# limuhit/pseudocylindrical_convolution

Hardware: AMD Instinct MI355X
Metric: ERP MPix/s enc+dec, 4096x2048 model-idx 3 (higher is better)
Workload: dtype f32; 1 GPU; ERP 4096x2048 encode+decode, model-idx 3 --ssim (valid_dim 56), 8 frame(s)/GPU/step; frames_per_gpu=8, parallelism=frames sharded, no data-path collective, weights=seeded random (transforms seed 1234, entropy randn*0.05 seed 7), content=smooth, cores_per_rank=16

## Files before the change

pseudocylindrical_convolution_amd/csrc/wino42.hip:

```cpp
#include <atomic>
#include <stdlib.h>
#include <type_traits>
#include "conv_host.h"

namespace {

#ifdef PCONV_W42_STAMP
__device__ unsigned long long w42_stamps[8][6];
#define W42_STAMP(var) const unsigned long long var = __builtin_readcyclecounter()
#else
#define W42_STAMP(var)
#endif

typedef float f32x16 __attribute__((ext_vector_type(16)));
typedef float f32x2 __attribute__((ext_vector_type(2)));
typedef __attribute__((address_space(3))) void lds_ptr_t;
typedef const __attribute__((address_space(1))) void glb_ptr_t;
typedef const __attribute__((address_space(1))) char glb_bytes_t;

constexpr int kThreads = 512, kWaves = 8;
constexpr int XW = 3;
constexpr int NXI = kWaves * XW;
constexpr int TX = 32, TY = 2;
constexpr int OROWS = 4 * TY, OCOLS = 2 * TX;
constexpr int CO = 64;
constexpr int KC = 4;
constexpr int PR = OROWS + 2, PC = OCOLS + 2;
constexpr int PSZ = KC * PR * PC;
constexpr int PLD = (PSZ + kThreads - 1) / kThreads;
constexpr int PBUF = PLD * kThreads;
constexpr int PRING = 2;
constexpr int NT = TX * TY;
constexpr int VSZ = NXI * KC * NT;
constexpr int USZ = KC * XW * CO;
constexpr int URING = 3;
constexpr int ULD = USZ / 4 / 64;
constexpr int UNROLL = 6;
constexpr int kStageFloats = PRING * PBUF + 2 * VSZ + kWaves * URING * USZ;
constexpr int kLdsFloats = kStageFloats + 256;
constexpr int ESZ = NXI * 16 * 32;
static_assert(2 * ESZ <= kStageFloats, "the two exchange buffers fit the stage memory");
static_assert(kLdsFloats * 4 <= 160 * 1024, "LDS of a CU");
static_assert(PSZ <= PBUF && USZ % 256 == 0, "stage sizes");
static_assert(PLD + 2 * ULD < 64, "vmcnt counts to 63");
static_assert(KC == 4 && NXI == 24, "transform: waves 0-3 take one channel of the stage each; three GEMMs per wave");

__global__ void wino42_pack_kernel(const float *__restrict__ w, float *__restrict__ upk, int cout, int cin, int cin_pad,
                                   int cblocks) {
  const long long total = (long long)cblocks * cin_pad * CO;
  const long long i = (long long)blockIdx.x * blockDim.x + threadIdx.x;
  if (i >= total) return;
  const int j = (int)(i % CO);
  const int ci = (int)((i / CO) % cin_pad);
  const int cb = (int)(i / ((long long)CO * cin_pad));
  const int co = cb * CO + j;
  float g[3][3];
#pragma unroll
  for (int a = 0; a < 3; a++)
#pragma unroll
    for (int b = 0; b < 3; b++) g[a][b] = (co < cout && ci < cin) ? w[(((size_t)co * cin + ci) * 3 + a) * 3 + b] : 0.f;
  float r[6][3];
#pragma unroll
  for (int b = 0; b < 3; b++) {
    const float g0 = g[0][b], g1 = g[1][b], g2 = g[2][b];
    r[0][b] = g0 * 0.25f;
    r[1][b] = (g0 + g1 + g2) * (-1.f / 6.f);
    r[2][b] = (g0 - g1 + g2) * (-1.f / 6.f);
    r[3][b] = g0 * (1.f / 24.f) + g1 * (1.f / 12.f) + g2 * (1.f / 6.f);
    r[4][b] = g0 * (1.f / 24.f) - g1 * (1.f / 12.f) + g2 * (1.f / 6.f);
    r[5][b] = g2;
  }
#pragma unroll
  for (int a = 0; a < 6; a++) {
    const float u[4] = {r[a][0], (r[a][0] + r[a][1] + r[a][2]) * 0.5f, (r[a][0] - r[a][1] + r[a][2]) * 0.5f, r[a][2]};
#pragma unroll
    for (int b = 0; b < 4; b++) {
      const int xi = a * 4 + b;
      upk[((((size_t)cb * kWaves + xi / XW) * cin_pad + ci) * XW + (xi % XW)) * CO + j] = u[b];
    }
  }
}

template <int OFF>
__device__ __forceinline__ float w42_lds_read(unsigned addr) {
  static_assert(OFF >= 0 && OFF < 65536, "ds_read offset field is 16 bits");
  float v;
  asm volatile("ds_read_b32 %0, %1 offset:%2" : "=v"(v) : "v"(addr), "n"(OFF));
  return v;
}

template <int PENDING>
__device__ __forceinline__ void w42_wait(float (&a)[2], float (&b)[2]) {
  asm volatile("s_waitcnt lgkmcnt(%4)" : "+v"(a[0]), "+v"(a[1]), "+v"(b[0]), "+v"(b[1]) : "n"(PENDING));
}

template <int U, int VB, int ST>
__device__ __forceinline__ void w42_read_step(float (&a)[2], float (&b)[2], unsigned abase, unsigned bbase) {
  constexpr int x = ST >> 1, kp = ST & 1;
  constexpr int aoff = (U * USZ + (kp * 2 * XW + x) * CO) * 4;
  constexpr int boff = (VB * VSZ + (x * KC + kp * 2) * NT) * 4;
  a[0] = w42_lds_read<aoff>(abase);
  a[1] = w42_lds_read<aoff + 128>(abase);
  b[0] = w42_lds_read<boff>(bbase);
  b[1] = w42_lds_read<boff + 128>(bbase);
}

struct W42Half {
  const float *tp;
  float *tv;
  float cf[3][5];
};
struct W42Rows {
  float t[5][4];
};
template <int PB>
__device__ __forceinline__ void w42_half_load(const W42Half &h, W42Rows &w) {
  const float *p = h.tp + PB * PBUF;
#pragma unroll
  for (int a = 0; a < 5; a++) {
    const f32x2 lo = *reinterpret_cast<const f32x2 *>(p + a * PC), hi = *reinterpret_cast<const f32x2 *>(p + a * PC + 2);
    w.t[a][0] = lo.x, w.t[a][1] = lo.y, w.t[a][2] = hi.x, w.t[a][3] = hi.y;
  }
}
__device__ __forceinline__ void w42_half_horizontal(W42Rows &w) {
#pragma unroll
  for (int a = 0; a < 5; a++) {
    const float d0 = w.t[a][0], d1 = w.t[a][1], d2 = w.t[a][2], d3 = w.t[a][3];
    w.t[a][0] = d0 - d2, w.t[a][1] = d1 + d2, w.t[a][2] = d2 - d1, w.t[a][3] = d1 - d3;
  }
}
template <int VBUF, int R>
__device__ __forceinline__ void w42_half_row(const W42Half &h, const W42Rows &w) {
  constexpr int XS = KC * NT;
  float *v = h.tv + VBUF * VSZ + R * 4 * XS;
#pragma unroll
  for (int j = 0; j < 4; j++) {
    float s = h.cf[R][4] * w.t[4][j];
    s = __builtin_fmaf(h.cf[R][3], w.t[3][j], s);
    s = __builtin_fmaf(h.cf[R][2], w.t[2][j], s);
    s = __builtin_fmaf(h.cf[R][1], w.t[1][j], s);
    s = __builtin_fmaf(h.cf[R][0], w.t[0][j], s);
    v[j * XS] = s;
  }
}

template <int U, int VB, int ST, bool IL, class PD, class WD>
__device__ __forceinline__ void w42_mma_steps(f32x16 (&acc)[XW][2][2], float (&a)[2][2], float (&b)[2][2], unsigned abase,
                                              unsigned bbase, const W42Half &h, W42Rows &rows, PD &pd, WD &wd) {
  constexpr int NST = 2 * XW;
  constexpr int X = ST >> 1, S = ST & 1;
  static_assert(NST == 6, "the transform pieces are placed by hand in six steps");
  if constexpr (ST + 1 < NST) w42_read_step<U, VB, ST + 1>(a[(ST + 1) & 1], b[(ST + 1) & 1], abase, bbase);
  w42_wait<(ST + 1 < NST) ? 4 : 0>(a[S], b[S]);
  __builtin_amdgcn_sched_barrier(0);
  using std::integral_constant;
  auto dma = [&](auto g_c) {
    constexpr int G = decltype(g_c)::value;
    if constexpr (IL && ST <= 1 && ST * 3 + G < PLD && G < 3) {
      __builtin_amdgcn_sched_barrier(0);
      pd(integral_constant<int, ST * 3 + G>{});
      __builtin_amdgcn_sched_barrier(0);
    }
    if constexpr (IL && ST == NST - 1 && G < ULD) {
      __builtin_amdgcn_sched_barrier(0);
      wd(integral_constant<int, G>{});
      __builtin_amdgcn_sched_barrier(0);
    }
  };
  acc[X][0][0] = __builtin_amdgcn_mfma_f32_32x32x2f32(a[S][0], b[S][0], acc[X][0][0], 0, 0, 0);
  if constexpr (ST == 0) {
    __builtin_amdgcn_sched_barrier(0);
    w42_half_load<VB ^ 1>(h, rows);
    __builtin_amdgcn_sched_barrier(0);
  }
  if constexpr (ST == 1) {
    __builtin_amdgcn_sched_barrier(0);
    w42_half_horizontal(rows);
    __builtin_amdgcn_sched_barrier(0);
  }
  dma(integral_constant<int, 0>{});
  acc[X][0][1] = __builtin_amdgcn_mfma_f32_32x32x2f32(a[S][0], b[S][1], acc[X][0][1], 0, 0, 0);
  dma(integral_constant<int, 1>{});
  acc[X][1][0] = __builtin_amdgcn_mfma_f32_32x32x2f32(a[S][1], b[S][0], acc[X][1][0], 0, 0, 0);
  if constexpr (ST >= 2 && ST <= 4) {
    __builtin_amdgcn_sched_barrier(0);
    w42_half_row<VB ^ 1, ST - 2>(h, rows);
    __builtin_amdgcn_sched_barrier(0);
  }
  dma(integral_constant<int, 2>{});
  acc[X][1][1] = __builtin_amdgcn_mfma_f32_32x32x2f32(a[S][1], b[S][1], acc[X][1][1], 0, 0, 0);
  __builtin_amdgcn_sched_barrier(0);
  if constexpr (ST + 1 < NST) w42_mma_steps<U, VB, ST + 1, IL>(acc, a, b, abase, bbase, h, rows, pd, wd);
}

template <bool RES, bool D2W>
__global__ __launch_bounds__(kThreads) void wino42_conv3x3_kernel(
    const float *__restrict__ in, const float *__restrict__ upk, float *out, int cin, int cin_pad, int h,
    int w, int cout, int ho, int wo, int tiles_r, int tiles_c, int cblocks, WView vin, WView vout, WEpilogue ep) {
  W42_STAMP(st_start);
  extern __shared__ float lds[];
  float *Ps = lds, *Vs = lds + PRING * PBUF, *Us = lds + PRING * PBUF + 2 * VSZ;

  int b = blockIdx.x;
  const int cb = b % cblocks;
  b /= cblocks;
  const int trx = b % tiles_r;
  b /= tiles_r;
  const int tcx = b % tiles_c;
  const int t = b / tiles_c;
  const int r0 = trx * OROWS, c0 = tcx * OCOLS, cout0 = cb * CO;

  const int tid = threadIdx.x;
  const int lane = tid & 63;
  const int wave = __builtin_amdgcn_readfirstlane(tid >> 6);
  const int l31 = lane & 31, half = lane >> 5;
  float *outp = out + (size_t)t * vout.ts;
  const int limit = ep.col_limit ? ep.col_limit[t % ep.npart] : wo;

  if (c0 >= limit) {
    for (int e = tid; e < CO * OROWS * OCOLS; e += kThreads) {
      const int col = e % OCOLS, row = (e / OCOLS) % OROWS, co = cout0 + e / (OCOLS * OROWS);
      if (co < cout && r0 + row < ho && c0 + col < wo) {
        if (D2W)
          outp[(size_t)(co >> 2) * vout.cs + (size_t)(2 * (r0 + row) + ((co >> 1) & 1)) * vout.rs + 2 * (c0 + col) + (co & 1)] = 0.f;
        else
          outp[(size_t)co * vout.cs + (size_t)(r0 + row) * vout.rs + c0 + col] = 0.f;
      }
    }
    return;
  }

  const float *inp = in + (size_t)t * vin.ts;
  const int nchunk = cin_pad / KC;

  unsigned xoffs[PLD];
#pragma unroll
  for (int j = 0; j < PLD; j++) {
    int e = tid + j * kThreads;
    e = e < PSZ ? e : 0;
    const int pc = e % PC, pr = (e / PC) % PR, ci = e / (PC * PR);
    int ir = r0 + pr, ic = c0 + pc;
    ir = ir < h ? ir : h - 1;
    ic = ic < w ? ic : w - 1;
    xoffs[j] = (unsigned)(((long long)ci * vin.cs + (long long)ir * vin.rs + ic) * 4);
  }
  const size_t xstep = (size_t)KC * vin.cs;
  auto patch_piece = [&](int chunk, int buf, int j) {
    unsigned xo = xoffs[j];
    asm volatile("" : "+v"(xo));
    glb_bytes_t *xb = (glb_bytes_t *)(inp + chunk * xstep);
    __builtin_amdgcn_global_load_lds((glb_ptr_t *)(xb + xo), (lds_ptr_t *)(Ps + buf * PBUF + j * kThreads + wave * 64), 4, 0,
                                     0);
  };
  auto issue_patch = [&](int chunk, int buf, bool guard) {
    if (guard && chunk >= nchunk) return;
#pragma unroll
    for (int j = 0; j < PLD; j++) patch_piece(chunk, buf, j);
  };
  const float *uw = upk + ((size_t)cb * kWaves + wave) * cin_pad * XW * CO;
  float *us_w = Us + wave * URING * USZ;
  auto weight_piece = [&](int chunk, auto j_c) {
    constexpr int j = decltype(j_c)::value;
    glb_bytes_t *src = (glb_bytes_t *)(uw + (size_t)chunk * USZ);
    float *dst = us_w + (chunk % URING) * USZ;
    unsigned lo = (unsigned)lane * 16u;
    asm volatile("" : "+v"(lo));
    __builtin_amdgcn_global_load_lds((glb_ptr_t *)(src + lo), (lds_ptr_t *)dst, 16, j * 1024, 0);
  };
  auto issue_weights = [&](int chunk, bool guard) {
    if (guard && chunk >= nchunk) return;
    static_assert(ULD == 3, "weight pieces are issued by name");
    weight_piece(chunk, std::integral_constant<int, 0>{});
    weight_piece(chunk, std::integral_constant<int, 1>{});
    weight_piece(chunk, std::integral_constant<int, 2>{});
  };

  const int wave4 = wave >> 2, tch = wave & 3;
  const int tty = lane >> 5, ttx = lane & 31;
  const float *tp0 = Ps + (tch * PR + 4 * tty + wave4) * PC + 2 * ttx;
  float *tv0 = Vs + (wave4 * 12 * KC + tch) * NT + lane;
  const W42Half half_t = {tp0, tv0,
                          {{wave4 ? -2.f : 4.f, wave4 ? -1.f : 0.f, wave4 ? 2.f : -5.f, wave4 ? 1.f : 0.f, wave4 ? 0.f : 1.f},
                           {wave4 ? 2.f : 0.f, wave4 ? -1.f : -4.f, wave4 ? -2.f : -4.f, 1.f, wave4 ? 0.f : 1.f},
                           {wave4 ? 4.f : 0.f, wave4 ? 0.f : 4.f, wave4 ? -5.f : -4.f, wave4 ? 0.f : -1.f, 1.f}}};
  auto transform_full = [&](int pbuf, int vbuf) {
    W42Rows rows;
    const float *p = tp0 + pbuf * PBUF;
#pragma unroll
    for (int a = 0; a < 5; a++) {
      const f32x2 lo = *reinterpret_cast<const f32x2 *>(p + a * PC), hi = *reinterpret_cast<const f32x2 *>(p + a * PC + 2);
      rows.t[a][0] = lo.x, rows.t[a][1] = lo.y, rows.t[a][2] = hi.x, rows.t[a][3] = hi.y;
    }
    w42_half_horizontal(rows);
    constexpr int XS = KC * NT;
    float *v = tv0 + vbuf * VSZ;
#pragma unroll
    for (int r = 0; r < 3; r++)
#pragma unroll
      for (int j = 0; j < 4; j++) {
        float s = half_t.cf[r][4] * rows.t[4][j];
        s = __builtin_fmaf(half_t.cf[r][3], rows.t[3][j], s);
        s = __builtin_fmaf(half_t.cf[r][2], rows.t[2][j], s);
        s = __builtin_fmaf(half_t.cf[r][1], rows.t[1][j], s);
        s = __builtin_fmaf(half_t.cf[r][0], rows.t[0][j], s);
        v[(r * 4 + j) * XS] = s;
      }
  };

  f32x16 acc[XW][2][2];
#pragma unroll
  for (int x = 0; x < XW; x++)
#pragma unroll
    for (int m = 0; m < 2; m++)
#pragma unroll
      for (int n = 0; n < 2; n++)
#pragma unroll
        for (int r = 0; r < 16; r++) acc[x][m][n][r] = 0.f;

  float *Bt = lds + kStageFloats;
  if (wave < 4) {
    const float *src = wave < 2 ? ep.bias : (ep.act == 1 ? ep.slope : nullptr);
    int co = cout0 + (wave & 1) * 64 + lane;
    co = co < cout ? co : cout - 1;
    if (src)
      __builtin_amdgcn_global_load_lds((glb_ptr_t *)(src + co), (lds_ptr_t *)(Bt + wave * 64), 4, 0, 0);
    else
      Bt[wave * 64 + lane] = 0.f;
  }
  issue_patch(0, 0, true);
#pragma unroll
  for (int k = 0; k < URING; k++) issue_weights(k, true);
  issue_patch(1, 1, true);
  __builtin_amdgcn_s_waitcnt(0);
  __syncthreads();
  transform_full(0, 0);

  const unsigned lds0 = (unsigned)reinterpret_cast<uintptr_t>(lds);
  const unsigned abase = lds0 + (unsigned)((us_w - lds) + half * XW * CO + l31) * 4u;
  const unsigned bbase = lds0 + (unsigned)((Vs - lds) + ((wave * XW) * KC + half) * NT + l31) * 4u;

#ifdef PCONV_W42_STAMP
  unsigned long long st_bar = 0, st_n = 0;
#endif
  W42_STAMP(st_prologue);
  auto body = [&](auto us_c, auto vb_c, auto steady_c, int chunk) {
    constexpr int US = decltype(us_c)::value;
    constexpr int vb = decltype(vb_c)::value;
    constexpr bool STEADY = decltype(steady_c)::value;
    W42_STAMP(tb0);
    if (STEADY)
      asm volatile("s_waitcnt vmcnt(%0) lgkmcnt(0)\n\ts_barrier" ::"n"(ULD) : "memory");
    else
      asm volatile("s_waitcnt vmcnt(0) lgkmcnt(0)\n\ts_barrier" ::: "memory");
#ifdef PCONV_W42_STAMP
    if (STEADY) st_bar += __builtin_readcyclecounter() - tb0, st_n += 1;
#endif
    if (!STEADY) issue_patch(chunk + 2, vb, true);
    float a[2][2], bv[2][2];
    W42Rows rows;
    w42_read_step<US, vb, 0>(a[0], bv[0], abase, bbase);
    auto pd = [&](auto j_c) {
      constexpr int J = decltype(j_c)::value;
      if (J * kThreads + wave * 64 >= PSZ) return;
      patch_piece(chunk + 2, vb, J);
    };
    auto wd = [&](auto j_c) { weight_piece(chunk + URING, j_c); };
    w42_mma_steps<US, vb, 0, STEADY>(acc, a, bv, abase, bbase, half_t, rows, pd, wd);
    asm volatile("s_waitcnt lgkmcnt(0)" ::: "memory");
    if (!STEADY) issue_weights(chunk + URING, true);
  };
  using std::integral_constant;
  auto group = [&](auto steady_c, int c6) {
    body(integral_constant<int, 0>{}, integral_constant<int, 0>{}, steady_c, c6);
    body(integral_constant<int, 1>{}, integral_constant<int, 1>{}, steady_c, c6 + 1);
    body(integral_constant<int, 2>{}, integral_constant<int, 0>{}, steady_c, c6 + 2);
    body(integral_constant<int, 0>{}, integral_constant<int, 1>{}, steady_c, c6 + 3);
    body(integral_constant<int, 1>{}, integral_constant<int, 0>{}, steady_c, c6 + 4);
    body(integral_constant<int, 2>{}, integral_constant<int, 1>{}, steady_c, c6 + 5);
  };
  int c6 = 0;
#pragma unroll 1
  for (; c6 + 2 * UNROLL <= nchunk; c6 += UNROLL) group(integral_constant<bool, true>{}, c6);
#pragma unroll 1
  for (; c6 < nchunk; c6 += UNROLL) group(integral_constant<bool, false>{}, c6);
  W42_STAMP(st_loop);
  __syncthreads();

  const int act = ep.act;
  const int trim_at = ep.trim ? limit : wo;
  const float *resp = RES ? ep.residual + (size_t)t * ep.vres.ts : nullptr;
  const int co16 = tid >> 5, etx = tid & 31;
  const int ocol = c0 + 2 * etx;
  struct ResBlock {
    f32x2 v[4];
  };
  auto load_res = [&](int k) {
    ResBlock rb = {{{0.f, 0.f}, {0.f, 0.f}, {0.f, 0.f}, {0.f, 0.f}}};
    if (RES && k < 8) {
      const int m = k >> 2, n = (k >> 1) & 1, hq = k & 1;
      const int oc = ocol < wo ? ocol : wo - 2;
      int co = cout0 + m * 32 + hq * 16 + co16;
      co = co < cout ? co : cout - 1;
#pragma unroll
      for (int a2 = 0; a2 < 4; a2++) {
        int rr = r0 + 4 * n + a2;
        rr = rr < ho ? rr : ho - 1;
        rb.v[a2] = *reinterpret_cast<const f32x2 *>(resp + (size_t)co * ep.vres.cs + (size_t)rr * ep.vres.rs + oc);
      }
    }
    return rb;
  };
  ResBlock rq[2] = {load_res(0), load_res(1)};
#pragma unroll
  for (int k = 0; k < 8; k++) {
    const int m = k >> 2, n = (k >> 1) & 1, hq = k & 1;
    float *Es = lds + (k & 1) * ESZ;
    const ResBlock rcur = rq[k & 1];
    rq[k & 1] = load_res(k + 2);
#pragma unroll
    for (int x = 0; x < XW; x++) {
      float *e = Es + ((wave * XW + x) * 16 + 4 * half) * 32 + l31;
#pragma unroll
      for (int rl = 0; rl < 8; rl++) e[((rl & 3) + 8 * (rl >> 2)) * 32] = acc[x][m][n][8 * hq + rl];
    }
    asm volatile("s_waitcnt lgkmcnt(0)\n\ts_barrier" ::: "memory");
    float mm[NXI];
#pragma unroll
    for (int xi = 0; xi < NXI; xi++) mm[xi] = Es[(xi * 16 + co16) * 32 + etx];
    const int row = m * 32 + hq * 16 + co16;
    const int co = cout0 + row;
    const int orow = r0 + 4 * n;
    if (co < cout && ocol < wo) {
      float s[6][2];
#pragma unroll
      for (int i = 0; i < 6; i++) {
        s[i][0] = mm[4 * i] + mm[4 * i + 1] + mm[4 * i + 2];
        s[i][1] = mm[4 * i + 1] - mm[4 * i + 2] - mm[4 * i + 3];
      }
      float y[4][2];
#pragma unroll
      for (int c = 0; c < 2; c++) {
        const float p12 = s[1][c] + s[2][c], m12 = s[1][c] - s[2][c];
        const float p34 = s[3][c] + s[4][c], m34 = s[3][c] - s[4][c];
        y[0][c] = s[0][c] + p12 + p34;
        y[1][c] = __builtin_fmaf(2.f, m34, m12);
        y[2][c] = __builtin_fmaf(4.f, p34, p12);
        y[3][c] = __builtin_fmaf(8.f, m34, m12) + s[5][c];
      }
      const float bco = Bt[row], sl = Bt[128 + row];
#pragma unroll
      for (int a2 = 0; a2 < 4; a2++) {
        if (orow + a2 >= ho) continue;
        float y0 = y[a2][0] + bco, y1 = y[a2][1] + bco;
        if (act == 1) {
          y0 = y0 < 0 ? y0 * sl : y0;
          y1 = y1 < 0 ? y1 * sl : y1;
        }
        if (RES) {
          y0 = rcur.v[a2].x + y0;
          y1 = rcur.v[a2].y + y1;
        }
        if (!D2W) {
          if (ocol >= trim_at) y0 = 0.f;
          if (ocol + 1 >= trim_at) y1 = 0.f;
          float *q = outp + (size_t)co * vout.cs + (size_t)(orow + a2) * vout.rs + ocol;
          f32x2 yv = {y0, y1};
          *reinterpret_cast<f32x2 *>(q) = yv;
        } else {
          float *q = outp + (size_t)(co >> 2) * vout.cs + (size_t)(2 * (orow + a2) + ((co >> 1) & 1)) * vout.rs + 2 * ocol +
                     (co & 1);
          q[0] = y0;
          q[2] = y1;
        }
      }
    }
  }
#ifdef PCONV_W42_STAMP
  if (blockIdx.x == gridDim.x / 2 + 1 && lane == 0) {
    unsigned long long *o = w42_stamps[wave];
    o[0] = st_start, o[1] = st_prologue, o[2] = st_loop, o[3] = __builtin_readcyclecounter(), o[4] = st_bar, o[5] = st_n;
  }
#endif
}

}

#ifdef PCONV_W42_STAMP
extern "C" int pconv_wino42_read_stamps(unsigned long long *out) {
  return hipMemcpyFromSymbol(out, HIP_SYMBOL(w42_stamps), sizeof(w42_stamps)) == hipSuccess ? 0 : 1;
}
#endif

extern "C" long long pconv_wino42_packed_size(int cout, int cin) {
  const int cblocks = (cout + CO - 1) / CO, cin_pad = (cin + KC - 1) / KC * KC;
  return (long long)cblocks * NXI * cin_pad * CO;
}

extern "C" int pconv_wino42_pack_weight(const float *w, float *packed, int cout, int cin, void *stream) {
  PCONV_REQUIRE(w && packed && cout > 0 && cin > 0, "wino42_pack: bad argument");
  const int cblocks = (cout + CO - 1) / CO, cin_pad = (cin + KC - 1) / KC * KC;
  const long long total = (long long)cblocks * cin_pad * CO;
  hipLaunchKernelGGL(wino42_pack_kernel, dim3((unsigned)((total + 255) / 256)), dim3(256), 0, as_stream(stream), w, packed,
                     cout, cin, cin_pad, cblocks);
  PCONV_LAUNCH_CHECK("wino42_pack_weight");
  return PCONV_OK;
}

extern "C" int pconv_wino42_supported(int cin, int h, int w, int cout, int d2w) {
  if (h < 6 || w < 4 || ((w - 2) & 1)) return 0;
  if (cin < 24 || cin % 24 || cout < 32) return 0;
  if (d2w && (cout & 3)) return 0;
  return 1;
}

extern "C" int pconv_conv3x3_wino42(const float *in, const float *packed_u, const float *bias, float *out, int tn, int cin,
                                    int h, int w, int cout, int act, const float *slope, const int32_t *col_limit,
                                    int npart, const float *residual, int trim, int d2w, const long long *views,
                                    void *stream) {
  WView vin, vout;
  WEpilogue ep;
  if (int rc = wino_check_args("conv3x3_wino42", pconv_wino42_supported, KC, true, in, packed_u, bias, out, cin, h, w, cout,
                               act, slope, col_limit, npart, residual, trim, d2w, views, &vin, &vout, &ep))
    return rc;
  const int ho = h - 2, wo = w - 2;
  const int tiles_r = (ho + OROWS - 1) / OROWS, tiles_c = (wo + OCOLS - 1) / OCOLS;
  const int cblocks = (cout + CO - 1) / CO, cin_pad = (cin + KC - 1) / KC * KC;
  const long long grid = (long long)tn * tiles_r * tiles_c * cblocks;
  PCONV_REQUIRE(grid > 0 && grid <= 0x7fffffffLL, "conv3x3_wino42: grid %lld out of range", grid);
  const size_t smem = (size_t)kLdsFloats * sizeof(float);
  using kernel_t = decltype(&wino42_conv3x3_kernel<false, false>);
  static const kernel_t kernels[3] = {wino42_conv3x3_kernel<false, false>, wino42_conv3x3_kernel<true, false>,
                                      wino42_conv3x3_kernel<false, true>};
  const int kind = d2w ? 2 : (residual ? 1 : 0);
  static std::atomic<unsigned long long> raised[3];
  if (int rc = pconv_raise_lds(kernels[kind], smem, raised[kind], "conv3x3_wino42")) return rc;
  hipLaunchKernelGGL(kernels[kind], dim3((unsigned)grid), dim3(kThreads), smem, as_stream(stream), in, packed_u, out, cin,
                     cin_pad, h, w, cout, ho, wo, tiles_r, tiles_c, cblocks, vin, vout, ep);
  PCONV_LAUNCH_CHECK("conv3x3_wino42");
  return PCONV_OK;
}
```

Measured before the change: 95.63 MPix/s.

## Add wide 128-output-channel Winograd F(4,3) tile variant for cout divisible by 128

Result: slower. 94.47 MPix/s (-1.2%).

```diff
diff --git a/pseudocylindrical_convolution_amd/csrc/wino42.hip b/pseudocylindrical_convolution_amd/csrc/wino42.hip
--- a/pseudocylindrical_convolution_amd/csrc/wino42.hip
+++ b/pseudocylindrical_convolution_amd/csrc/wino42.hip
@@ -6,7 +6,7 @@
 namespace {
 
 #ifdef PCONV_W42_STAMP
-__device__ unsigned long long w42_stamps[8][6];
+__device__ unsigned long long w42_stamps[2][8][6];
 #define W42_STAMP(var) const unsigned long long var = __builtin_readcyclecounter()
 #else
 #define W42_STAMP(var)
@@ -21,32 +21,55 @@
 constexpr int kThreads = 512, kWaves = 8;
 constexpr int XW = 3;
 constexpr int NXI = kWaves * XW;
-constexpr int TX = 32, TY = 2;
-constexpr int OROWS = 4 * TY, OCOLS = 2 * TX;
-constexpr int CO = 64;
+constexpr int TY = 2;
+constexpr int OROWS = 4 * TY;
+constexpr int BCOLS = 64;
 constexpr int KC = 4;
-constexpr int PR = OROWS + 2, PC = OCOLS + 2;
-constexpr int PSZ = KC * PR * PC;
-constexpr int PLD = (PSZ + kThreads - 1) / kThreads;
-constexpr int PBUF = PLD * kThreads;
+constexpr int PR = OROWS + 2;
 constexpr int PRING = 2;
-constexpr int NT = TX * TY;
-constexpr int VSZ = NXI * KC * NT;
-constexpr int USZ = KC * XW * CO;
-constexpr int URING = 3;
-constexpr int ULD = USZ / 4 / 64;
-constexpr int UNROLL = 6;
-constexpr int kStageFloats = PRING * PBUF + 2 * VSZ + kWaves * URING * USZ;
+constexpr int ESZ = NXI * 16 * 32;
+
+template <bool WIDE>
+struct W42Geom {
+  static constexpr int CO = WIDE ? 128 : 64;
+  static constexpr int TX = WIDE ? 16 : 32;
+  static constexpr int MT = CO / 32, NB = TX * TY / 32;
+  static constexpr int OCOLS = 2 * TX;
+  static constexpr int PC = OCOLS + 2;
+  static constexpr int PSZ = KC * PR * PC;
+  static constexpr int PLD = (PSZ + kThreads - 1) / kThreads;
+  static constexpr int PBUF = PLD * kThreads;
+  static constexpr int NT = TX * TY;
+  static constexpr int VSZ = NXI * KC * NT;
+  static constexpr int USZ = KC * XW * CO;
+  static constexpr int URING = WIDE ? 2 : 3;
+  static constexpr int ULD = USZ / 4 / 64;
+  static constexpr int UNROLL = WIDE ? 2 : 6;
+  static constexpr int kStageFloats = PRING * PBUF + 2 * VSZ + kWaves * URING * USZ;
+  static_assert(MT * NB == 4, "four MFMAs per step");
+  static_assert(2 * ESZ <= kStageFloats, "the two exchange buffers fit the stage memory");
+  static_assert(PSZ <= PBUF && USZ % 256 == 0 && ULD % 3 == 0, "stage sizes");
+  static_assert(PLD <= 6 && PLD + 2 * ULD < 64, "patch pieces fit two steps; vmcnt counts to 63");
+};
+constexpr int kStageFloats = W42Geom<false>::kStageFloats;
 constexpr int kLdsFloats = kStageFloats + 256;
-constexpr int ESZ = NXI * 16 * 32;
-static_assert(2 * ESZ <= kStageFloats, "the two exchange buffers fit the stage memory");
+static_assert(W42Geom<true>::kStageFloats <= kStageFloats, "one LDS size for both shapes");
 static_assert(kLdsFloats * 4 <= 160 * 1024, "LDS of a CU");
-static_assert(PSZ <= PBUF && USZ % 256 == 0, "stage sizes");
-static_assert(PLD + 2 * ULD < 64, "vmcnt counts to 63");
 static_assert(KC == 4 && NXI == 24, "transform: waves 0-3 take one channel of the stage each; three GEMMs per wave");
 
+__host__ __device__ inline int w42_wide_blocks(int cout) { return cout % 128 == 0 ? cout / 128 : 0; }
+struct W42Slice {
+  size_t off;
+  int pitch;
+};
+__host__ __device__ inline W42Slice w42_slice64(int cb, int nwide, int cin_pad) {
+  if (nwide) return {(size_t)(cb >> 1) * NXI * cin_pad * 128 + (size_t)(cb & 1) * 64, 128};
+  return {(size_t)cb * NXI * cin_pad * 64, 64};
+}
+
 __global__ void wino42_pack_kernel(const float *__restrict__ w, float *__restrict__ upk, int cout, int cin, int cin_pad,
-                                   int cblocks) {
+                                   int cblocks, int nwide) {
+  constexpr int CO = 64;
   const long long total = (long long)cblocks * cin_pad * CO;
   const long long i = (long long)blockIdx.x * blockDim.x + threadIdx.x;
   if (i >= total) return;
@@ -54,6 +77,7 @@
   const int ci = (int)((i / CO) % cin_pad);
   const int cb = (int)(i / ((long long)CO * cin_pad));
   const int co = cb * CO + j;
+  const W42Slice sl = w42_slice64(cb, nwide, cin_pad);
   float g[3][3];
 #pragma unroll
   for (int a = 0; a < 3; a++)
@@ -76,7 +100,7 @@
 #pragma unroll
     for (int b = 0; b < 4; b++) {
       const int xi = a * 4 + b;
-      upk[((((size_t)cb * kWaves + xi / XW) * cin_pad + ci) * XW + (xi % XW)) * CO + j] = u[b];
+      upk[sl.off + (((size_t)(xi / XW) * cin_pad + ci) * XW + (xi % XW)) * sl.pitch + j] = u[b];
     }
   }
 }
@@ -93,131 +117,186 @@
 __device__ __forceinline__ void w42_wait(float (&a)[2], float (&b)[2]) {
   asm volatile("s_waitcnt lgkmcnt(%4)" : "+v"(a[0]), "+v"(a[1]), "+v"(b[0]), "+v"(b[1]) : "n"(PENDING));
 }
-
-template <int U, int VB, int ST>
-__device__ __forceinline__ void w42_read_step(float (&a)[2], float (&b)[2], unsigned abase, unsigned bbase) {
+template <int PENDING>
+__device__ __forceinline__ void w42_wait(float (&a)[4], float (&b)[1]) {
+  asm volatile("s_waitcnt lgkmcnt(%5)" : "+v"(a[0]), "+v"(a[1]), "+v"(a[2]), "+v"(a[3]), "+v"(b[0]) : "n"(PENDING));
+}
+
+template <bool WIDE, int U, int VB, int ST>
+__device__ __forceinline__ void w42_read_step(float (&a)[W42Geom<WIDE>::MT], float (&b)[W42Geom<WIDE>::NB], unsigned abase,
+                                              unsigned bbase) {
+  using G = W42Geom<WIDE>;
   constexpr int x = ST >> 1, kp = ST & 1;
-  constexpr int aoff = (U * USZ + (kp * 2 * XW + x) * CO) * 4;
-  constexpr int boff = (VB * VSZ + (x * KC + kp * 2) * NT) * 4;
+  constexpr int aoff = (U * G::USZ + (kp * 2 * XW + x) * G::CO) * 4;
+  constexpr int boff = (VB * G::VSZ + (x * KC + kp * 2) * G::NT) * 4;
   a[0] = w42_lds_read<aoff>(abase);
   a[1] = w42_lds_read<aoff + 128>(abase);
-  b[0] = w42_lds_read<boff>(bbase);
-  b[1] = w42_lds_read<boff + 128>(bbase);
-}
-
+  if constexpr (WIDE) {
+    a[2] = w42_lds_read<aoff + 256>(abase);
+    a[3] = w42_lds_read<aoff + 384>(abase);
+    b[0] = w42_lds_read<boff>(bbase);
+  } else {
+    b[0] = w42_lds_read<boff>(bbase);
+    b[1] = w42_lds_read<boff + 128>(bbase);
+  }
+}
+
+template <bool WIDE>
 struct W42Half {
   const float *tp;
   float *tv;
   float cf[3][5];
 };
+template <>
+struct W42Half<true> {
+  const float *tp;
+  float *tv[2];
+  float cf[3][5];
+  float sg;
+  bool jh;
+};
+template <bool WIDE>
 struct W42Rows {
-  float t[5][4];
+  float t[5][WIDE ? 3 : 4];
 };
-template <int PB>
-__device__ __forceinline__ void w42_half_load(const W42Half &h, W42Rows &w) {
-  const float *p = h.tp + PB * PBUF;
+template <bool WIDE, int PB>
+__device__ __forceinline__ void w42_half_load(const W42Half<WIDE> &h, W42Rows<WIDE> &w) {
+  using G = W42Geom<WIDE>;
+  const float *p = h.tp + PB * G::PBUF;
 #pragma unroll
   for (int a = 0; a < 5; a++) {
-    const f32x2 lo = *reinterpret_cast<const f32x2 *>(p + a * PC), hi = *reinterpret_cast<const f32x2 *>(p + a * PC + 2);
-    w.t[a][0] = lo.x, w.t[a][1] = lo.y, w.t[a][2] = hi.x, w.t[a][3] = hi.y;
-  }
-}
-__device__ __forceinline__ void w42_half_horizontal(W42Rows &w) {
+    if constexpr (WIDE) {
+      w.t[a][0] = p[a * G::PC], w.t[a][1] = p[a * G::PC + 1], w.t[a][2] = p[a * G::PC + 2];
+    } else {
+      const f32x2 lo = *reinterpret_cast<const f32x2 *>(p + a * G::PC), hi = *reinterpret_cast<const f32x2 *>(p + a * G::PC + 2);
+      w.t[a][0] = lo.x, w.t[a][1] = lo.y, w.t[a][2] = hi.x, w.t[a][3] = hi.y;
+    }
+  }
+}
+__device__ __forceinline__ void w42_half_horizontal(const W42Half<false> &, W42Rows<false> &w) {
 #pragma unroll
   for (int a = 0; a < 5; a++) {
     const float d0 = w.t[a][0], d1 = w.t[a][1], d2 = w.t[a][2], d3 = w.t[a][3];
     w.t[a][0] = d0 - d2, w.t[a][1] = d1 + d2, w.t[a][2] = d2 - d1, w.t[a][3] = d1 - d3;
   }
 }
-template <int VBUF, int R>
-__device__ __forceinline__ void w42_half_row(const W42Half &h, const W42Rows &w) {
-  constexpr int XS = KC * NT;
-  float *v = h.tv + VBUF * VSZ + R * 4 * XS;
-#pragma unroll
-  for (int j = 0; j < 4; j++) {
-    float s = h.cf[R][4] * w.t[4][j];
-    s = __builtin_fmaf(h.cf[R][3], w.t[3][j], s);
-    s = __builtin_fmaf(h.cf[R][2], w.t[2][j], s);
-    s = __builtin_fmaf(h.cf[R][1], w.t[1][j], s);
-    s = __builtin_fmaf(h.cf[R][0], w.t[0][j], s);
-    v[j * XS] = s;
-  }
-}
-
-template <int U, int VB, int ST, bool IL, class PD, class WD>
-__device__ __forceinline__ void w42_mma_steps(f32x16 (&acc)[XW][2][2], float (&a)[2][2], float (&b)[2][2], unsigned abase,
-                                              unsigned bbase, const W42Half &h, W42Rows &rows, PD &pd, WD &wd) {
+__device__ __forceinline__ void w42_half_horizontal(const W42Half<true> &h, W42Rows<true> &w) {
+#pragma unroll
+  for (int a = 0; a < 5; a++) {
+    const float e0 = w.t[a][0], e1 = w.t[a][1], e2 = w.t[a][2];
+    w.t[a][0] = e0 - e2, w.t[a][1] = __builtin_fmaf(h.sg, h.jh ? e0 : e2, e1);
+  }
+}
+template <bool WIDE, int R>
+__device__ __forceinline__ float w42_half_value(const W42Half<WIDE> &h, const W42Rows<WIDE> &w, int j) {
+  float s = h.cf[R][4] * w.t[4][j];
+  s = __builtin_fmaf(h.cf[R][3], w.t[3][j], s);
+  s = __builtin_fmaf(h.cf[R][2], w.t[2][j], s);
+  s = __builtin_fmaf(h.cf[R][1], w.t[1][j], s);
+  s = __builtin_fmaf(h.cf[R][0], w.t[0][j], s);
+  return s;
+}
+template <bool WIDE, int VBUF, int R>
+__device__ __forceinline__ void w42_half_row(const W42Half<WIDE> &h, const W42Rows<WIDE> &w) {
+  using G = W42Geom<WIDE>;
+  constexpr int XS = KC * G::NT;
+  if constexpr (WIDE) {
+#pragma unroll
+    for (int j = 0; j < 2; j++) h.tv[j][VBUF * G::VSZ + R * 4 * XS] = w42_half_value<WIDE, R>(h, w, j);
+  } else {
+    float *v = h.tv + VBUF * G::VSZ + R * 4 * XS;
+#pragma unroll
+    for (int j = 0; j < 4; j++) v[j * XS] = w42_half_value<WIDE, R>(h, w, j);
+  }
+}
+
+template <bool WIDE, int U, int VB, int ST, bool IL, class PD, class WD>
+__device__ __forceinline__ void w42_mma_steps(f32x16 (&acc)[XW][W42Geom<WIDE>::MT][W42Geom<WIDE>::NB],
+                                              float (&a)[2][W42Geom<WIDE>::MT], float (&b)[2][W42Geom<WIDE>::NB],
+                                              unsigned abase, unsigned bbase, const W42Half<WIDE> &h, W42Rows<WIDE> &rows,
+                                              PD &pd, WD &wd) {
+  using G = W42Geom<WIDE>;
   constexpr int NST = 2 * XW;
   constexpr int X = ST >> 1, S = ST & 1;
+  constexpr int UPG = G::ULD / 3;
   static_assert(NST == 6, "the transform pieces are placed by hand in six steps");
-  if constexpr (ST + 1 < NST) w42_read_step<U, VB, ST + 1>(a[(ST + 1) & 1], b[(ST + 1) & 1], abase, bbase);
-  w42_wait<(ST + 1 < NST) ? 4 : 0>(a[S], b[S]);
+  if constexpr (ST + 1 < NST) w42_read_step<WIDE, U, VB, ST + 1>(a[(ST + 1) & 1], b[(ST + 1) & 1], abase, bbase);
+  w42_wait<(ST + 1 < NST) ? G::MT + G::NB : 0>(a[S], b[S]);
   __builtin_amdgcn_sched_barrier(0);
   using std::integral_constant;
   auto dma = [&](auto g_c) {
-    constexpr int G = decltype(g_c)::value;
-    if constexpr (IL && ST <= 1 && ST * 3 + G < PLD && G < 3) {
+    constexpr int GP = decltype(g_c)::value;
+    if constexpr (IL && ST <= 1 && ST * 3 + GP < G::PLD && GP < 3) {
       __builtin_amdgcn_sched_barrier(0);
-      pd(integral_constant<int, ST * 3 + G>{});
+      pd(integral_constant<int, ST * 3 + GP>{});
       __builtin_amdgcn_sched_barrier(0);
     }
-    if constexpr (IL && ST == NST - 1 && G < ULD) {
+    if constexpr (IL && ST == NST - 1 && GP < 3) {
       __builtin_amdgcn_sched_barrier(0);
-      wd(integral_constant<int, G>{});
+      wd(integral_constant<int, GP * UPG>{});
+      if constexpr (UPG == 2) wd(integral_constant<int, GP * UPG + 1>{});
       __builtin_amdgcn_sched_barrier(0);
     }
   };
-  acc[X][0][0] = __builtin_amdgcn_mfma_f32_32x32x2f32(a[S][0], b[S][0], acc[X][0][0], 0, 0, 0);
+  auto mma = [&](auto q_c) {
+    constexpr int Q = decltype(q_c)::value;
+    constexpr int m = WIDE ? Q : Q >> 1, n = WIDE ? 0 : Q & 1;
+    acc[X][m][n] = __builtin_amdgcn_mfma_f32_32x32x2f32(a[S][m], b[S][n], acc[X][m][n], 0, 0, 0);
+  };
+  mma(integral_constant<int, 0>{});
   if constexpr (ST == 0) {
     __builtin_amdgcn_sched_barrier(0);
-    w42_half_load<VB ^ 1>(h, rows);
+    w42_half_load<WIDE, VB ^ 1>(h, rows);
     __builtin_amdgcn_sched_barrier(0);
   }
   if constexpr (ST == 1) {
     __builtin_amdgcn_sched_barrier(0);
-    w42_half_horizontal(rows);
+    w42_half_horizontal(h, rows);
     __builtin_amdgcn_sched_barrier(0);
   }
   dma(integral_constant<int, 0>{});
-  acc[X][0][1] = __builtin_amdgcn_mfma_f32_32x32x2f32(a[S][0], b[S][1], acc[X][0][1], 0, 0, 0);
+  mma(integral_constant<int, 1>{});
   dma(integral_constant<int, 1>{});
-  acc[X][1][0] = __builtin_amdgcn_mfma_f32_32x32x2f32(a[S][1], b[S][0], acc[X][1][0], 0, 0, 0);
+  mma(integral_constant<int, 2>{});
   if constexpr (ST >= 2 && ST <= 4) {
     __builtin_amdgcn_sched_barrier(0);
-    w42_half_row<VB ^ 1, ST - 2>(h, rows);
+    w42_half_row<WIDE, VB ^ 1, ST - 2>(h, rows);
     __builtin_amdgcn_sched_barrier(0);
   }
   dma(integral_constant<int, 2>{});
-  acc[X][1][1] = __builtin_amdgcn_mfma_f32_32x32x2f32(a[S][1], b[S][1], acc[X][1][1], 0, 0, 0);
+  mma(integral_constant<int, 3>{});
   __builtin_amdgcn_sched_barrier(0);
-  if constexpr (ST + 1 < NST) w42_mma_steps<U, VB, ST + 1, IL>(acc, a, b, abase, bbase, h, rows, pd, wd);
-}
-
-template <bool RES, bool D2W>
-__global__ __launch_bounds__(kThreads) void wino42_conv3x3_kernel(
-    const float *__restrict__ in, const float *__restrict__ upk, float *out, int cin, int cin_pad, int h,
-    int w, int cout, int ho, int wo, int tiles_r, int tiles_c, int cblocks, WView vin, WView vout, WEpilogue ep) {
+  if constexpr (ST + 1 < NST) w42_mma_steps<WIDE, U, VB, ST + 1, IL>(acc, a, b, abase, bbase, h, rows, pd, wd);
+}
+
+struct W42Block {
+  const float *inp;
+  const float *uw0;
+  float *outp;
+  int t, r0, c0, cout0;
+  bool dead;
+  int limit;
+  bool stamp;
+};
+
+template <bool WIDE, int UPITCH, bool RES, bool D2W>
+__device__ __forceinline__ void w42_workgroup(const W42Block &blk, float *lds, int cin_pad, int h, int w, int cout, int ho,
+                                              int wo, const WView &vin, const WView &vout, const WEpilogue &ep) {
+  using G = W42Geom<WIDE>;
+  constexpr int CO = G::CO, OCOLS = G::OCOLS, PC = G::PC, PSZ = G::PSZ, PLD = G::PLD, PBUF = G::PBUF, NT = G::NT;
+  constexpr int VSZ = G::VSZ, USZ = G::USZ, URING = G::URING, ULD = G::ULD, UNROLL = G::UNROLL, MT = G::MT, NB = G::NB;
   W42_STAMP(st_start);
-  extern __shared__ float lds[];
   float *Ps = lds, *Vs = lds + PRING * PBUF, *Us = lds + PRING * PBUF + 2 * VSZ;
-
-  int b = blockIdx.x;
-  const int cb = b % cblocks;
-  b /= cblocks;
-  const int trx = b % tiles_r;
-  b /= tiles_r;
-  const int tcx = b % tiles_c;
-  const int t = b / tiles_c;
-  const int r0 = trx * OROWS, c0 = tcx * OCOLS, cout0 = cb * CO;
+  const int r0 = blk.r0, c0 = blk.c0, cout0 = blk.cout0, t = blk.t;
 
   const int tid = threadIdx.x;
   const int lane = tid & 63;
   const int wave = __builtin_amdgcn_readfirstlane(tid >> 6);
   const int l31 = lane & 31, half = lane >> 5;
-  float *outp = out + (size_t)t * vout.ts;
-  const int limit = ep.col_limit ? ep.col_limit[t % ep.npart] : wo;
-
-  if (c0 >= limit) {
+  float *outp = blk.outp;
+  const int limit = blk.limit;
+
+  if (blk.dead || c0 >= wo) {
     for (int e = tid; e < CO * OROWS * OCOLS; e += kThreads) {
       const int col = e % OCOLS, row = (e / OCOLS) % OROWS, co = cout0 + e / (OCOLS * OROWS);
       if (co < cout && r0 + row < ho && c0 + col < wo) {
@@ -230,7 +309,7 @@
     return;
   }
 
-  const float *inp = in + (size_t)t * vin.ts;
+  const float *inp = blk.inp;
   const int nchunk = cin_pad / KC;
 
   unsigned xoffs[PLD];
@@ -257,63 +336,72 @@
 #pragma unroll
     for (int j = 0; j < PLD; j++) patch_piece(chunk, buf, j);
   };
-  const float *uw = upk + ((size_t)cb * kWaves + wave) * cin_pad * XW * CO;
+  constexpr int upitch = UPITCH;
+  static_assert(UPITCH >= CO && (UPITCH == 64 || UPITCH == 128), "rows of the packed weights");
+  const float *uw = blk.uw0 + (size_t)wave * cin_pad * XW * upitch;
   float *us_w = Us + wave * URING * USZ;
   auto weight_piece = [&](int chunk, auto j_c) {
     constexpr int j = decltype(j_c)::value;
-    glb_bytes_t *src = (glb_bytes_t *)(uw + (size_t)chunk * USZ);
-    float *dst = us_w + (chunk % URING) * USZ;
-    unsigned lo = (unsigned)lane * 16u;
+    constexpr int jo = j & 3, jb = j - jo;
+    glb_bytes_t *src = (glb_bytes_t *)(uw + (size_t)chunk * (KC * XW) * upitch) + (WIDE ? jb * 1024 : j * (16 * upitch - 1024));
+    float *dst = us_w + (chunk % URING) * USZ + jb * 256;
+    unsigned lo = UPITCH == CO ? (unsigned)lane * 16u : (unsigned)(lane >> 4) * (unsigned)(UPITCH * 4) + (unsigned)(lane & 15) * 16u;
     asm volatile("" : "+v"(lo));
-    __builtin_amdgcn_global_load_lds((glb_ptr_t *)(src + lo), (lds_ptr_t *)dst, 16, j * 1024, 0);
+    __builtin_amdgcn_global_load_lds((glb_ptr_t *)(src + lo), (lds_ptr_t *)dst, 16, jo * 1024, 0);
   };
   auto issue_weights = [&](int chunk, bool guard) {
     if (guard && chunk >= nchunk) return;
-    static_assert(ULD == 3, "weight pieces are issued by name");
+    static_assert(ULD == 3 || ULD == 6, "weight pieces are issued by name");
     weight_piece(chunk, std::integral_constant<int, 0>{});
     weight_piece(chunk, std::integral_constant<int, 1>{});
     weight_piece(chunk, std::integral_constant<int, 2>{});
+    if constexpr (ULD == 6) {
+      weight_piece(chunk, std::integral_constant<int, 3>{});
+      weight_piece(chunk, std::integral_constant<int, 4>{});
+      weight_piece(chunk, std::integral_constant<int, 5>{});
+    }
   };
 
   const int wave4 = wave >> 2, tch = wave & 3;
-  const int tty = lane >> 5, ttx = lane & 31;
-  const float *tp0 = Ps + (tch * PR + 4 * tty + wave4) * PC + 2 * ttx;
-  float *tv0 = Vs + (wave4 * 12 * KC + tch) * NT + lane;
-  const W42Half half_t = {tp0, tv0,
-                          {{wave4 ? -2.f : 4.f, wave4 ? -1.f : 0.f, wave4 ? 2.f : -5.f, wave4 ? 1.f : 0.f, wave4 ? 0.f : 1.f},
-                           {wave4 ? 2.f : 0.f, wave4 ? -1.f : -4.f, wave4 ? -2.f : -4.f, 1.f, wave4 ? 0.f : 1.f},
-                           {wave4 ? 4.f : 0.f, wave4 ? 0.f : 4.f, wave4 ? -5.f : -4.f, wave4 ? 0.f : -1.f, 1.f}}};
-  auto transform_full = [&](int pbuf, int vbuf) {
-    W42Rows rows;
-    const float *p = tp0 + pbuf * PBUF;
-#pragma unroll
-    for (int a = 0; a < 5; a++) {
-      const f32x2 lo = *reinterpret_cast<const f32x2 *>(p + a * PC), hi = *reinterpret_cast<const f32x2 *>(p + a * PC + 2);
-      rows.t[a][0] = lo.x, rows.t[a][1] = lo.y, rows.t[a][2] = hi.x, rows.t[a][3] = hi.y;
-    }
-    w42_half_horizontal(rows);
-    constexpr int XS = KC * NT;
-    float *v = tv0 + vbuf * VSZ;
+  W42Half<WIDE> half_t;
+  if constexpr (WIDE) {
+    const int tty = lane >> 5, jh = (lane >> 4) & 1, ttx = lane & 15;
+    half_t.tp = Ps + (tch * PR + 4 * tty + wave4) * PC + 2 * ttx + jh;
+    float *tv0 = Vs + (wave4 * 12 * KC + tch) * NT + tty * 16 + ttx;
+    half_t.tv[0] = tv0 + (jh ? 3 : 0) * KC * NT;
+    half_t.tv[1] = tv0 + (jh ? 2 : 1) * KC * NT;
+    half_t.sg = jh ? -1.f : 1.f;
+    half_t.jh = jh != 0;
+  } else {
+    const int tty = lane >> 5, ttx = lane & 31;
+    half_t.tp = Ps + (tch * PR + 4 * tty + wave4) * PC + 2 * ttx;
+    half_t.tv = Vs + (wave4 * 12 * KC + tch) * NT + lane;
+  }
+  {
+    const float cf[3][5] = {{wave4 ? -2.f : 4.f, wave4 ? -1.f : 0.f, wave4 ? 2.f : -5.f, wave4 ? 1.f : 0.f, wave4 ? 0.f : 1.f},
+                            {wave4 ? 2.f : 0.f, wave4 ? -1.f : -4.f, wave4 ? -2.f : -4.f, 1.f, wave4 ? 0.f : 1.f},
+                            {wave4 ? 4.f : 0.f, wave4 ? 0.f : 4.f, wave4 ? -5.f : -4.f, wave4 ? 0.f : -1.f, 1.f}};
 #pragma unroll
     for (int r = 0; r < 3; r++)
 #pragma unroll
-      for (int j = 0; j < 4; j++) {
-        float s = half_t.cf[r][4] * rows.t[4][j];
-        s = __builtin_fmaf(half_t.cf[r][3], rows.t[3][j], s);
-        s = __builtin_fmaf(half_t.cf[r][2], rows.t[2][j], s);
-        s = __builtin_fmaf(half_t.cf[r][1], rows.t[1][j], s);
-        s = __builtin_fmaf(half_t.cf[r][0], rows.t[0][j], s);
-        v[(r * 4 + j) * XS] = s;
-      }
-  };
-
-  f32x16 acc[XW][2][2];
+      for (int a = 0; a < 5; a++) half_t.cf[r][a] = cf[r][a];
+  }
+  auto transform_full = [&]() {
+    W42Rows<WIDE> rows;
+    w42_half_load<WIDE, 0>(half_t, rows);
+    w42_half_horizontal(half_t, rows);
+    w42_half_row<WIDE, 0, 0>(half_t, rows);
+    w42_half_row<WIDE, 0, 1>(half_t, rows);
+    w42_half_row<WIDE, 0, 2>(half_t, rows);
+  };
+
+  f32x16 acc[XW][MT][NB];
 #pragma unroll
   for (int x = 0; x < XW; x++)
 #pragma unroll
-    for (int m = 0; m < 2; m++)
-#pragma unroll
-      for (int n = 0; n < 2; n++)
+    for (int m = 0; m < MT; m++)
+#pragma unroll
+      for (int n = 0; n < NB; n++)
 #pragma unroll
         for (int r = 0; r < 16; r++) acc[x][m][n][r] = 0.f;
 
@@ -333,7 +421,7 @@
   issue_patch(1, 1, true);
   __builtin_amdgcn_s_waitcnt(0);
   __syncthreads();
-  transform_full(0, 0);
+  transform_full();
 
   const unsigned lds0 = (unsigned)reinterpret_cast<uintptr_t>(lds);
   const unsigned abase = lds0 + (unsigned)((us_w - lds) + half * XW * CO + l31) * 4u;
@@ -356,54 +444,67 @@
     if (STEADY) st_bar += __builtin_readcyclecounter() - tb0, st_n += 1;
 #endif
     if (!STEADY) issue_patch(chunk + 2, vb, true);
-    float a[2][2], bv[2][2];
-    W42Rows rows;
-    w42_read_step<US, vb, 0>(a[0], bv[0], abase, bbase);
+    float a[2][MT], bv[2][NB];
+    W42Rows<WIDE> rows;
+    w42_read_step<WIDE, US, vb, 0>(a[0], bv[0], abase, bbase);
     auto pd = [&](auto j_c) {
       constexpr int J = decltype(j_c)::value;
       if (J * kThreads + wave * 64 >= PSZ) return;
       patch_piece(chunk + 2, vb, J);
     };
     auto wd = [&](auto j_c) { weight_piece(chunk + URING, j_c); };
-    w42_mma_steps<US, vb, 0, STEADY>(acc, a, bv, abase, bbase, half_t, rows, pd, wd);
+    w42_mma_steps<WIDE, US, vb, 0, STEADY>(acc, a, bv, abase, bbase, half_t, rows, pd, wd);
     asm volatile("s_waitcnt lgkmcnt(0)" ::: "memory");
     if (!STEADY) issue_weights(chunk + URING, true);
   };
   using std::integral_constant;
-  auto group = [&](auto steady_c, int c6) {
-    body(integral_constant<int, 0>{}, integral_constant<int, 0>{}, steady_c, c6);
-    body(integral_constant<int, 1>{}, integral_constant<int, 1>{}, steady_c, c6 + 1);
-    body(integral_constant<int, 2>{}, integral_constant<int, 0>{}, steady_c, c6 + 2);
-    body(integral_constant<int, 0>{}, integral_constant<int, 1>{}, steady_c, c6 + 3);
-    body(integral_constant<int, 1>{}, integral_constant<int, 0>{}, steady_c, c6 + 4);
-    body(integral_constant<int, 2>{}, integral_constant<int, 1>{}, steady_c, c6 + 5);
-  };
-  int c6 = 0;
+  auto group = [&](auto steady_c, int c0g) {
+    if constexpr (UNROLL == 6) {
+      body(integral_constant<int, 0>{}, integral_constant<int, 0>{}, steady_c, c0g);
+      body(integral_constant<int, 1>{}, integral_constant<int, 1>{}, steady_c, c0g + 1);
+      body(integral_constant<int, 2>{}, integral_constant<int, 0>{}, steady_c, c0g + 2);
+      body(integral_constant<int, 0>{}, integral_constant<int, 1>{}, steady_c, c0g + 3);
+      body(integral_constant<int, 1>{}, integral_constant<int, 0>{}, steady_c, c0g + 4);
+      body(integral_constant<int, 2>{}, integral_constant<int, 1>{}, steady_c, c0g + 5);
+    } else {
+      static_assert(UNROLL == 2 && URING == 2, "ring slot = buffer");
+      body(integral_constant<int, 0>{}, integral_constant<int, 0>{}, steady_c, c0g);
+      body(integral_constant<int, 1>{}, integral_constant<int, 1>{}, steady_c, c0g + 1);
+    }
+  };
+  int cg = 0;
 #pragma unroll 1
-  for (; c6 + 2 * UNROLL <= nchunk; c6 += UNROLL) group(integral_constant<bool, true>{}, c6);
+  for (; cg + 2 * UNROLL <= nchunk; cg += UNROLL) group(integral_constant<bool, true>{}, cg);
 #pragma unroll 1
-  for (; c6 < nchunk; c6 += UNROLL) group(integral_constant<bool, false>{}, c6);
+  for (; cg < nchunk; cg += UNROLL) group(integral_constant<bool, false>{}, cg);
   W42_STAMP(st_loop);
   __syncthreads();
 
   const int act = ep.act;
   const int trim_at = ep.trim ? limit : wo;
   const float *resp = RES ? ep.residual + (size_t)t * ep.vres.ts : nullptr;
-  const int co16 = tid >> 5, etx = tid & 31;
+  const int co16 = tid >> 5, et = tid & 31;
+  const int etx = WIDE ? et & 15 : et, ety = WIDE ? et >> 4 : 0;
   const int ocol = c0 + 2 * etx;
+  auto round_of = [](int k, int &m, int &n, int &hq) {
+    hq = k & 1;
+    m = WIDE ? k >> 1 : k >> 2;
+    n = WIDE ? 0 : (k >> 1) & 1;
+  };
   struct ResBlock {
     f32x2 v[4];
   };
   auto load_res = [&](int k) {
     ResBlock rb = {{{0.f, 0.f}, {0.f, 0.f}, {0.f, 0.f}, {0.f, 0.f}}};
     if (RES && k < 8) {
-      const int m = k >> 2, n = (k >> 1) & 1, hq = k & 1;
+      int m, n, hq;
+      round_of(k, m, n, hq);
       const int oc = ocol < wo ? ocol : wo - 2;
       int co = cout0 + m * 32 + hq * 16 + co16;
       co = co < cout ? co : cout - 1;
 #pragma unroll
       for (int a2 = 0; a2 < 4; a2++) {
-        int rr = r0 + 4 * n + a2;
+        int rr = r0 + 4 * (n + ety) + a2;
         rr = rr < ho ? rr : ho - 1;
         rb.v[a2] = *reinterpret_cast<const f32x2 *>(resp + (size_t)co * ep.vres.cs + (size_t)rr * ep.vres.rs + oc);
       }
@@ -413,7 +514,8 @@
   ResBlock rq[2] = {load_res(0), load_res(1)};
 #pragma unroll
   for (int k = 0; k < 8; k++) {
-    const int m = k >> 2, n = (k >> 1) & 1, hq = k & 1;
+    int m, n, hq;
+    round_of(k, m, n, hq);
     float *Es = lds + (k & 1) * ESZ;
     const ResBlock rcur = rq[k & 1];
     rq[k & 1] = load_res(k + 2);
@@ -426,10 +528,10 @@
     asm volatile("s_waitcnt lgkmcnt(0)\n\ts_barrier" ::: "memory");
     float mm[NXI];
 #pragma unroll
-    for (int xi = 0; xi < NXI; xi++) mm[xi] = Es[(xi * 16 + co16) * 32 + etx];
+    for (int xi = 0; xi < NXI; xi++) mm[xi] = Es[(xi * 16 + co16) * 32 + et];
     const int row = m * 32 + hq * 16 + co16;
     const int co = cout0 + row;
-    const int orow = r0 + 4 * n;
+    const int orow = r0 + 4 * (n + ety);
     if (co < cout && ocol < wo) {
       float s[6][2];
 #pragma unroll
@@ -476,11 +578,46 @@
     }
   }
 #ifdef PCONV_W42_STAMP
-  if (blockIdx.x == gridDim.x / 2 + 1 && lane == 0) {
-    unsigned long long *o = w42_stamps[wave];
+  if (blk.stamp && lane == 0) {
+    unsigned long long *o = w42_stamps[WIDE][wave];
     o[0] = st_start, o[1] = st_prologue, o[2] = st_loop, o[3] = __builtin_readcyclecounter(), o[4] = st_bar, o[5] = st_n;
   }
 #endif
+}
+
+enum { W42_WIDE = 0, W42_64 = 1, W42_64_OF_128 = 2 };
+template <bool RES, bool D2W, int MODE>
+__global__ __launch_bounds__(kThreads) void wino42_conv3x3_kernel(
+    const float *__restrict__ in, const float *__restrict__ upk, float *out, int cin, int cin_pad, int h,
+    int w, int cout, int ho, int wo, int tiles_r, int tiles_c, int cblocks, WView vin, WView vout, WEpilogue ep) {
+  extern __shared__ float lds[];
+  const int nwide = cblocks / 2;
+  const int units = MODE == W42_WIDE ? 2 * nwide : cblocks;
+  int b = blockIdx.x;
+  const int u = b % units;
+  b /= units;
+  const int trx = b % tiles_r;
+  b /= tiles_r;
+  const int tcx = b % tiles_c;
+  const int t = b / tiles_c;
+  const int limit = ep.col_limit ? ep.col_limit[t % ep.npart] : wo;
+  W42Block blk;
+  blk.inp = in + (size_t)t * vin.ts;
+  blk.outp = out + (size_t)t * vout.ts;
+  blk.t = t, blk.r0 = trx * OROWS, blk.limit = limit;
+  blk.dead = tcx * BCOLS >= limit;
+  blk.stamp = blockIdx.x == gridDim.x / 2 + 1;
+  if constexpr (MODE == W42_WIDE) {
+    const int cbw = u % nwide, side = u / nwide;
+    blk.c0 = tcx * BCOLS + side * W42Geom<true>::OCOLS, blk.cout0 = cbw * 128;
+    blk.uw0 = upk + (size_t)cbw * NXI * cin_pad * 128;
+    w42_workgroup<true, 128, RES, D2W>(blk, lds, cin_pad, h, w, cout, ho, wo, vin, vout, ep);
+  } else {
+    const W42Slice sl = w42_slice64(u, MODE == W42_64_OF_128 ? nwide : 0, cin_pad);
+    blk.c0 = tcx * BCOLS, blk.cout0 = u * 64;
+    blk.uw0 = upk + sl.off;
+    w42_workgroup<false, MODE == W42_64_OF_128 ? 128 : 64, RES, D2W>(blk, lds, cin_pad, h, w, cout, ho, wo, vin, vout, ep);
+  }
 }
 
 }
@@ -492,16 +629,16 @@
 #endif
 
 extern "C" long long pconv_wino42_packed_size(int cout, int cin) {
-  const int cblocks = (cout + CO - 1) / CO, cin_pad = (cin + KC - 1) / KC * KC;
-  return (long long)cblocks * NXI * cin_pad * CO;
+  const int cblocks = (cout + 63) / 64, cin_pad = (cin + KC - 1) / KC * KC;
+  return (long long)cblocks * NXI * cin_pad * 64;
 }
 
 extern "C" int pconv_wino42_pack_weight(const float *w, float *packed, int cout, int cin, void *stream) {
   PCONV_REQUIRE(w && packed && cout > 0 && cin > 0, "wino42_pack: bad argument");
-  const int cblocks = (cout + CO - 1) / CO, cin_pad = (cin + KC - 1) / KC * KC;
-  const long long total = (long long)cblocks * cin_pad * CO;
+  const int cblocks = (cout + 63) / 64, cin_pad = (cin + KC - 1) / KC * KC;
+  const long long total = (long long)cblocks * cin_pad * 64;
   hipLaunchKernelGGL(wino42_pack_kernel, dim3((unsigned)((total + 255) / 256)), dim3(256), 0, as_stream(stream), w, packed,
-                     cout, cin, cin_pad, cblocks);
+                     cout, cin, cin_pad, cblocks, w42_wide_blocks(cout));
   PCONV_LAUNCH_CHECK("wino42_pack_weight");
   return PCONV_OK;
 }
@@ -523,16 +660,21 @@
                                act, slope, col_limit, npart, residual, trim, d2w, views, &vin, &vout, &ep))
     return rc;
   const int ho = h - 2, wo = w - 2;
-  const int tiles_r = (ho + OROWS - 1) / OROWS, tiles_c = (wo + OCOLS - 1) / OCOLS;
-  const int cblocks = (cout + CO - 1) / CO, cin_pad = (cin + KC - 1) / KC * KC;
-  const long long grid = (long long)tn * tiles_r * tiles_c * cblocks;
+  const int tiles_r = (ho + OROWS - 1) / OROWS, tiles_c = (wo + BCOLS - 1) / BCOLS;
+  const int cblocks = (cout + 63) / 64, cin_pad = (cin + KC - 1) / KC * KC;
+  const char *env = getenv("PCONV_W42_WIDE");
+  const int nwide = w42_wide_blocks(cout);
+  const int mode = !nwide ? W42_64 : (env && atoi(env) == 0) ? W42_64_OF_128 : W42_WIDE;
+  const int units = mode == W42_WIDE ? 2 * nwide : cblocks;
+  const long long grid = (long long)tn * tiles_r * tiles_c * units;
   PCONV_REQUIRE(grid > 0 && grid <= 0x7fffffffLL, "conv3x3_wino42: grid %lld out of range", grid);
   const size_t smem = (size_t)kLdsFloats * sizeof(float);
-  using kernel_t = decltype(&wino42_conv3x3_kernel<false, false>);
-  static const kernel_t kernels[3] = {wino42_conv3x3_kernel<false, false>, wino42_conv3x3_kernel<true, false>,
-                                      wino42_conv3x3_kernel<false, true>};
-  const int kind = d2w ? 2 : (residual ? 1 : 0);
-  static std::atomic<unsigned long long> raised[3];
+  using kernel_t = decltype(&wino42_conv3x3_kernel<false, false, W42_WIDE>);
+#define W42_KINDS(MODE) wino42_conv3x3_kernel<false, false, MODE>, wino42_conv3x3_kernel<true, false, MODE>, wino42_conv3x3_kernel<false, true, MODE>
+  static const kernel_t kernels[9] = {W42_KINDS(W42_WIDE), W42_KINDS(W42_64), W42_KINDS(W42_64_OF_128)};
+#undef W42_KINDS
+  const int kind = (d2w ? 2 : (residual ? 1 : 0)) + 3 * mode;
+  static std::atomic<unsigned long long> raised[9];
   if (int rc = pconv_raise_lds(kernels[kind], smem, raised[kind], "conv3x3_wino42")) return rc;
   hipLaunchKernelGGL(kernels[kind], dim3((unsigned)grid), dim3(kThreads), smem, as_stream(stream), in, packed_u, out, cin,
                      cin_pad, h, w, cout, ho, wo, tiles_r, tiles_c, cblocks, vin, vout, ep);
```
